# NoSuchThingAsRandom/EpidemicSimulator

Hardware: AMD Instinct MI355X
Metric: citizen-timesteps/sec (higher is better)
Workload: dtype u32 citizen word; u32 uniform vs ceil(q*2^32) (reference: f64 uniform; tolerance 2^-32 per draw); 1 GPU; uk64m: 64000000 citizens, 290000 Output Areas, 10 seeds, steps 1..667 of 5000, interventions on; seed=1592598545

## Files before the change

### epidemicsimulator_amd/csrc/esim_chunk_sets.h

```cpp
#pragma once
#include "esim_kernels_common.h"
#define IV_VALID   0x80000000u
#define IV_PT      (1u << 14)
#define IV_HW      (1u << 15)
#define IV_AS_WORK (1u << 16)
__device__ __forceinline__ uint32_t iv_present(uint32_t iv, uint32_t j, const Decision &q)
{
    if (!(iv & IV_VALID) || j < (iv & 127u) || j > ((iv >> 7) & 127u)) return 0u;
    if (q.bus_dir && (iv & IV_PT)) return 0u;
    const bool at_work = q.at_work && (iv & IV_HW);
    return ((iv & IV_AS_WORK) != 0u) == at_work ? 1u : 0u;
}

__device__ __forceinline__ uint32_t status_in_chunk(const Dev &d, uint32_t w, uint32_t t0, uint32_t j)
{
    const uint32_t f = CW_VAX_REL(w);
    if (f != CW_VAX_NONE && j > f) return ESIM_VACCINATED;
    return status_of(CW_TE(w), t0 + j, d.exposed_time, d.infected_time);
}

__device__ __forceinline__ uint32_t where_in_step(const Dev &d, uint32_t w, uint32_t t0, uint32_t j, const Decision &q)
{
    if (status_in_chunk(d, w, t0, j) != ESIM_INFECTED) return 0u;
    if (q.bus_dir && (w & FL_USES_PT)) return 4u;
    return (q.at_work && (w & FL_HAS_WORK)) ? 2u : 1u;
}

#define FX(x, i) ((uint32_t)__builtin_amdgcn_readlane((int)(x), (int)(i)))
struct M96 { unsigned long long lo; uint32_t hi; };
__device__ __forceinline__ M96 m96_and(M96 a, M96 b) { return M96{ a.lo & b.lo, a.hi & b.hi }; }
__device__ __forceinline__ M96 m96_andn(M96 a, M96 b) { return M96{ a.lo & ~b.lo, a.hi & ~b.hi }; }
__device__ __forceinline__ bool m96_any(M96 a) { return a.lo != 0ull || a.hi != 0u; }
__device__ __forceinline__ M96 m96_range(uint32_t a, uint32_t b)
{
    M96 r = { 0ull, 0u };
    if (a < 64u) { const uint32_t e = min(b, 63u); r.lo = (e == 63u ? ~0ull : ((1ull << (e + 1u)) - 1ull)) & (~0ull << a); }
    if (b >= 64u) { const uint32_t s0 = a > 64u ? a - 64u : 0u, e = min(b - 64u, 31u); r.hi = (e == 31u ? ~0u : ((1u << (e + 1u)) - 1u)) & (~0u << s0); }
    return r;
// ... 61 lines not shown
```

### epidemicsimulator_amd/csrc/esim_device.h

```cpp
#pragma once
#include <stdint.h>

#define CW_TE_SHIFT    19u
#define CW_BUS_EXPOSED (1u << 18)
#define CW_FLAGS       0xFFu
#define CW_VAX_SHIFT   11u
#define CW_VAX_MASK    (0x7Fu << CW_VAX_SHIFT)
#define CW_KEEP        (CW_FLAGS | CW_VAX_MASK)
#define CW_VAX_NONE    0xFFFFFFFFu
#define CW_PLAN_SKIP   (1u << 10)
#define CW_VAX_REL(w)  ((((w) >> CW_VAX_SHIFT) & 0x7Fu) ? 127u - (((w) >> CW_VAX_SHIFT) & 0x7Fu) : CW_VAX_NONE)
#define CW_VAX_FIELD(j) ((127u - (j)) << CW_VAX_SHIFT)
#define CW_TE(w)       ((w) >> CW_TE_SHIFT)
#define CW_MAKE(te, rest) (((te) << CW_TE_SHIFT) | (rest))
#define TE_SUSCEPTIBLE 0x1FFFu
#define TE_VACCINATED  0x1FFEu
#define TE_RECOVERED   0x1FFDu
#define TE_BIAS        512u
#define TE_SLOTS       8192u
#define ESIM_MAX_STEP  7600u

#define FL_USES_PT        0x01u
#define FL_MASK_COMPLIANT 0x02u
#define FL_SAME_AREA      0x04u
// ... 47 lines not shown
    uint32_t prev_cut;
    uint32_t prev_n, prev_n_eff, prev_vax;
    uint32_t vax_cuts;
    uint32_t vax_planned, prev_planned;
    uint32_t xs_need;
    uint32_t xs_need_all;
    uint32_t vax_fail;
    uint32_t err_where;
    uint32_t peer_error;
    uint32_t quiet;
    uint32_t chunk_bus;
    uint32_t replan_from;
    uint32_t repair_ran;
    uint32_t vax_repairs;
};

#define ERR_FIELD(code) ((code) ? 1u << (5u * (((code) < 1u || (code) > 6u ? 6u : (code)) - 1u)) : 0u)
#define ERR_MAX_WORLD 31u
#define XE_WORDS (2u + ERR_MAX_WORLD)
static inline __host__ __device__ uint32_t err_decode(uint32_t word)
{
    for (uint32_t c = 1u; c <= 6u; ++c) if ((word >> (5u * (c - 1u))) & 31u) return c;
    return word ? 6u : 0u;
}

struct UnitRec { uint32_t slot, link, lo, n_mem, code, own, m_first, pad; };

struct BldRec { uint32_t res_lo, res_hi, wrk_lo, wrk_hi, type, ovf_lo, ovf_hi, pad; };
#define SD_REPL 8u

struct ItemRec { uint32_t id, a_lo, a_hi, b_lo, b_hi, aux, link, own; };
#define CHUNK_WAVES_MAX 4096u
#define SLOT_COUNTERS_ONLY 0x40000000u
#ifndef ITEM_RECS
#define ITEM_RECS 7u
#define SLOT_IV_STRIDE 8u
#endif
#define LANE_STATE 24u
#define LANE_HSLOT 25u

struct Decision {
    uint32_t lockdown;
    uint32_t mask;
    uint32_t at_work, bus_dir;
};

struct Dev {
    uint32_t n;
    uint32_t n_global;
    uint32_t id_base;
    uint32_t n_bld, n_room, n_pt;
    uint32_t *cit;
    const uint32_t *home, *work, *room;
    const uint32_t *res_off, *res_idx;
    const uint32_t *wrk_off, *wrk_idx;
    const uint32_t *room_off, *room_idx;
    const uint32_t *room_bld;
    const uint8_t  *bld_type;
    uint32_t *cnt_bld[MARK_SLOTS];
    uint32_t *cnt_room[MARK_SLOTS];
    uint32_t *touched_bld[MARK_SLOTS], *touched_room[MARK_SLOTS], *touched_route[MARK_SLOTS], *touched_route_big[MARK_SLOTS];
    uint32_t *route_flag[MARK_SLOTS];
    uint32_t *exp_step;
    uint32_t *exp_part;
    struct Decision *dec;
    unsigned long long *hkey;
    uint32_t hcap;
    uint32_t *hitems;
    struct ItemRec *item_rec;
    uint32_t *slot_state;
    uint32_t *slot_iv;
    uint32_t *vec;
    uint32_t items_cap;
    struct UnitRec *units;
    uint32_t *route_pairs;
    uint32_t *pair_cnt;
    uint32_t *used_cnt;
    uint32_t *route_pairs_big;
    uint32_t big_pairs_cap;
    const uint32_t *ovf_off;
    uint32_t ovf_room_base;
    uint32_t *ovf;
    uint32_t ovf_n;
    uint32_t n_wrk_idx, n_room_idx;
    const int32_t *sch_of_bld;
    uint32_t n_sch;
    uint32_t *sch_diff;
    const uint4 *where4;
    const struct BldRec *bld8;
    uint32_t *big_list;
    uint32_t big_qcap;
    uint32_t *used_pref;
    uint32_t unit_qcap;
    uint32_t *newexp;
    uint32_t newexp_cap;
    uint32_t *hot;
    uint32_t *cursor;
    uint32_t max_route;
    uint32_t *vax_ev;
    uint32_t *vax_cnt;
    uint32_t *vax_now;
    uint32_t *lost_list;
    uint32_t *vax_delta;
    uint32_t *xf_adj;
    uint32_t *hist;
    uint32_t *log;
    uint32_t *log_off;
    const uint64_t *thr;
    Ctrl *ctrl;
    struct esim_step_result *records;
    uint32_t n_routes;
    const uint32_t *route_off;
    const uint32_t *route_riders;
    const uint32_t *route_of;
    uint32_t *bus_key; uint32_t *bus_idx; uint32_t *bus_cnt; uint8_t *bus_flag;
    uint32_t exposed_time, infected_time, vaccination_rate, bus_capacity, start_hour, end_hour;
    uint32_t seed_lo, seed_hi;
    double thr_lockdown, thr_vacc, thr_mask_pt, thr_mask_all;
    uint32_t max_steps;
    uint32_t n_shards;
    uint32_t n_shared_bld, n_shared_room;
// ... 58 lines not shown
```

### epidemicsimulator_amd/csrc/esim_host_upload.h

```cpp
namespace {

struct UploadHost {
    const esim_population *pop;
    uint32_t N, B, R, n_global;
    bool sharded;
    std::vector<uint8_t> fl;
    std::vector<uint32_t> room_fixed;
    std::vector<uint32_t> route_off, riders, route_of;
    uint32_t n_routes = 0, max_route = 0, n_big_routes = 0;
    bool any_big = false;
    std::vector<uint32_t> res_off, res_idx, wrk_off, wrk_idx, room_off, room_idx;
    bool home_sorted = true;
};

int upload_validate(esim_ctx_impl *c, UploadHost &u)
{
    const esim_population *pop = u.pop; const uint32_t N = u.N, B = u.B, R = u.R;
    if (!pop->home_building || !pop->work_building || !pop->room || !pop->flags || !pop->building_area || !pop->building_type)
        return fail(c, ESIM_EINVAL, "esim_upload_population: a required array is NULL");
    if (R && !pop->room_building) return fail(c, ESIM_EINVAL, "esim_upload_population: room_building is NULL");
    if (pop->n_seeds && !pop->seeds) return fail(c, ESIM_EINVAL, "esim_upload_population: seeds is NULL");
    u.n_global = pop->n_citizens_global ? pop->n_citizens_global : N;
    if ((uint64_t)pop->citizen_id_base + N > u.n_global) return fail(c, ESIM_EINVAL, "esim_upload_population: shard range exceeds n_citizens_global");
    u.sharded = u.n_global != N || pop->n_shared_buildings || pop->n_shared_rooms;
// ... 156 lines not shown
    if ((rc = dev_alloc_fill(c, &d.item_rec, d.items_cap))) return rc;
    if ((rc = dev_alloc_fill(c, &d.vec, (size_t)cap * FREE_MAX))) return rc;
    if ((rc = dev_alloc_fill(c, &d.slot_state, cap))) return rc;
    if ((rc = dev_alloc_fill(c, &d.slot_iv, (size_t)cap * SLOT_IV_STRIDE))) return rc;
    size_t units = 0;
    auto add_lists = [&](const std::vector<uint32_t> &off) {
        for (size_t i = 0; i + 1 < off.size(); ++i) {
            const size_t pairs = (size_t)(off[i + 1] - off[i]) * FREE_MAX;
            if (pairs > UNIT_INLINE) units += (pairs + UNIT_PAIRS - 1) / UNIT_PAIRS;
        }
    };
    add_lists(u.res_off); add_lists(u.wrk_off); add_lists(u.room_off);
    units = std::min<size_t>(units, (size_t)N / 8u + 65536u);
    d.unit_qcap = (uint32_t)std::max<size_t>(1024, units * 2u / SUBQ);
    if ((rc = dev_alloc_fill(c, &d.units, (size_t)d.unit_qcap * SUBQ, 0xFF))) return rc;
    if ((rc = dev_alloc_fill(c, &d.route_pairs, (size_t)d.items_cap * (CHUNK_BUS_STEPS / 4u)))) return rc;
    d.big_pairs_cap = (uint32_t)std::max<size_t>(1, std::min<size_t>((size_t)d.items_cap / 4u, u.n_big_routes) * CHUNK_BUS_STEPS);
    if ((rc = dev_alloc_fill(c, &d.route_pairs_big, d.big_pairs_cap))) return rc;
    std::vector<uint32_t> sch_members((size_t)B + 1, 0);
    for (uint32_t i = 0; i < N; ++i) if (u.fl[i] & FL_WORK_SCHOOL) sch_members[pop->work_building[i] + 1]++;
    for (uint32_t b = 0; b < B; ++b) sch_members[b + 1] += sch_members[b];
    std::vector<uint32_t> ovf_off(u.res_off.size());
    for (size_t i = 0; i < u.res_off.size(); ++i) ovf_off[i] = u.res_off[i] + u.wrk_off[i] + sch_members[i];
    if ((rc = dev_upload(c, &d.ovf_off, ovf_off.data(), ovf_off.size()))) return rc;
    {
        std::vector<int32_t> sch_of(B ? B : 1, -1);
        uint32_t n_sch = 0;
        for (uint32_t b = 0; b < B; ++b) if (pop->building_type[b] == ESIM_SCHOOL) sch_of[b] = (int32_t)n_sch++;
        d.n_sch = n_sch;
        if ((rc = dev_upload(c, &d.sch_of_bld, sch_of.data(), sch_of.size()))) return rc;
    }
    {
        std::vector<uint4> w4(N ? N : 1);
        for (uint32_t i = 0; i < N; ++i) w4[i] = make_uint4(pop->home_building[i], pop->work_building[i], u.room_fixed[i], u.route_of[i]);
        if ((rc = dev_upload(c, &d.where4, w4.data(), w4.size()))) return rc;
        std::vector<BldRec> b8(B ? B : 1);
        for (uint32_t b = 0; b < B; ++b) b8[b] = BldRec{ u.res_off[b], u.res_off[b + 1], u.wrk_off[b], u.wrk_off[b + 1], (uint32_t)pop->building_type[b], ovf_off[b], ovf_off[b + 1], 0u };
        if ((rc = dev_upload(c, &d.bld8, b8.data(), b8.size()))) return rc;
        if ((rc = dev_alloc_fill(c, &d.sch_diff, (size_t)(d.n_sch ? d.n_sch : 1) * SD_REPL * 2u * FREE_MAX))) return rc;
    }
    d.ovf_room_base = ovf_off.back();
    d.ovf_n = d.ovf_room_base + u.room_off.back() + 1u;
    if ((rc = dev_alloc_fill(c, &d.ovf, (size_t)d.ovf_n))) return rc;
    d.n_wrk_idx = (uint32_t)u.wrk_idx.size(); d.n_room_idx = (uint32_t)u.room_idx.size();
    d.big_qcap = d.items_cap / SUBQ;
    if ((rc = dev_alloc_fill(c, &d.big_list, (size_t)d.big_qcap * SUBQ * 3u))) return rc;
    if ((rc = dev_alloc_fill(c, &d.used_pref, CHUNK_WAVES_MAX + 1u))) return rc;
    if ((rc = dev_alloc_fill(c, &d.pair_cnt, 16384u)) || (rc = dev_alloc_fill(c, &d.used_cnt, 16384u))) return rc;
    if ((rc = dev_alloc_fill(c, &d.hot, (size_t)HOT_COUNT * HOT_STRIDE))) return rc;
    d.newexp_cap = N / SUBQ + 1u;
    if ((rc = dev_alloc_fill(c, &d.newexp, (size_t)d.newexp_cap * SUBQ))) return rc;
    if ((rc = dev_alloc_fill(c, &d.cursor, (size_t)EXP_ROWS * FREE_MAX))) return rc;
    return ESIM_OK;
}

int upload_step_tables(esim_ctx_impl *c, const UploadHost &u)
{
    const uint32_t N = u.N, B = u.B, R = u.R;
    Dev &d = c->d; int rc;
    const size_t per_parity = (size_t)B + R + u.n_routes;
    for (int p = 0; p < (int)MARK_SLOTS; ++p) {
        uint32_t *base = c->cnt_base + p * per_parity;
        d.cnt_bld[p] = base; d.cnt_room[p] = base + B; d.route_flag[p] = base + B + R;
        if ((rc = dev_alloc(c, &d.touched_bld[p], B)) || (rc = dev_alloc(c, &d.touched_room[p], R))) return rc;
        if ((rc = dev_alloc(c, &d.touched_route[p], u.n_routes)) || (rc = dev_alloc(c, &d.touched_route_big[p], u.n_routes))) return rc;
    }
    if ((rc = dev_alloc(c, &d.vax_ev, (size_t)FREE_MAX * VACC_MAX_RATE))) return rc;
// ... 268 lines not shown
```

### epidemicsimulator_amd/csrc/esim_kernels_common.h

```cpp
#pragma once
#include <hip/hip_runtime.h>
#include "../../include/esim.h"
#include "esim_device.h"
#include "philox.h"

#define TPB 256
#define FIN_TPB 1024

__device__ __forceinline__ uint32_t status_of(uint32_t te, uint32_t t, uint32_t et, uint32_t it)
{
    if (te == TE_SUSCEPTIBLE) return ESIM_SUSCEPTIBLE;
    if (te == TE_VACCINATED) return ESIM_VACCINATED;
    if (te == TE_RECOVERED) return ESIM_RECOVERED;
    uint32_t d = t + TE_BIAS - te;
    if (d <= et) return ESIM_EXPOSED;
    if (d <= et + 1u + it) return ESIM_INFECTED;
    return ESIM_RECOVERED;
}

__device__ __forceinline__ uint32_t ld(const uint32_t *p)
{
    return __hip_atomic_load(p, __ATOMIC_RELAXED, __HIP_MEMORY_SCOPE_AGENT);
}

// ... 73 lines not shown
#ifdef ESIM_WAVE_PROFILE
#define PROF_ROW 16u
#define PROF_NOW() ((uint32_t)wall_clock64())
#define PROF_PUT(d, i, v) do { if ((threadIdx.x & 63u) == 0) (d).prof_buf[(size_t)(((blockIdx.x * TPB + threadIdx.x) >> 6)) * PROF_ROW + (i)] = (uint32_t)(v); } while (0)
#define BOOKS_PROF(d, i, v) do { if (threadIdx.x == 0) (d).prof_buf[(size_t)16383 * PROF_ROW + (i)] = (uint32_t)(v); } while (0)
#define TINY_PROF(d, i) do { if (threadIdx.x == 0) (d).prof_buf[(size_t)16382 * PROF_ROW + (i)] = (uint32_t)wall_clock64(); } while (0)
#else
#define BOOKS_PROF(d, i, v) do { (void)sizeof(v); } while (0)
#define TINY_PROF(d, i) do { } while (0)
#define PROF_NOW() 0u
#define PROF_PUT(d, i, v) do { (void)sizeof(v); } while (0)
#endif


#ifdef ESIM_COUNT_WORK
enum { WK_ENTRIES = 0,
       WK_KEYS,
       WK_CLAIMS,
       WK_RECORDS,
       WK_DIRECT,
       WK_FOLDED,
       WK_ITEMS,
       WK_MEMBERS,
       WK_MEMBERS_IDX,
       WK_PAIRS,
       WK_PAIRS_ACTIVE,
       WK_BLOCKS,
       WK_DRAWS,
       WK_UNITS,
       WK_ROUTE_PAIRS,
       WK_RIDERS,
       WK_BUS_DRAWS,
       WK_HITS,
       WK_N };
#define WORK_TALLY uint32_t wk_[WK_N]; for (int wk_i = 0; wk_i < WK_N; ++wk_i) wk_[wk_i] = 0u
#define WORK_ADD(i, x) (wk_[i] += (uint32_t)(x))
#define WORK_FLUSH(d) do { for (int wk_i = 0; wk_i < WK_N; ++wk_i) { uint32_t x_ = wk_[wk_i]; for (int o_ = 32; o_ > 0; o_ >>= 1) x_ += __shfl_xor(x_, o_, 64); \
        if ((threadIdx.x & 63u) == 0 && x_) atomicAdd(&(d).work_cnt[wk_i], (unsigned long long)x_); wk_[wk_i] = 0u; } } while (0)
#define WORK_ARG , uint32_t *wk_
#define WORK_PASS , wk_
#else
#define WORK_TALLY do { } while (0)
#define WORK_ADD(i, x) do { } while (0)
#define WORK_FLUSH(d) do { } while (0)
#define WORK_ARG
#define WORK_PASS
#endif
```

### epidemicsimulator_amd/csrc/esim_kernels_draw.h

```cpp
#pragma once
#include "esim_kernels_common.h"
#include "esim_rank.h"
#include "esim_chunk_sets.h"
#include "esim_kernels_marks.h"
__device__ __forceinline__ void expose_min(const Dev &d, Ctrl *ctrl, uint32_t m, uint32_t w, uint32_t s, uint32_t bus)
{
    const uint32_t cand = CW_MAKE(s + TE_BIAS, bus | (w & CW_KEEP));
    const uint32_t prev = atomicMin(&d.cit[m], cand);
    if (bus && cand < prev && CW_VAX_REL(w) != CW_VAX_NONE) {
        const uint32_t at = atomicAdd(&d.hot[HOT_LOST * HOT_STRIDE], 1u);
        if (at < LOST_CAP) d.lost_list[at] = m;
    }
    if (cand < prev && CW_TE(prev) == TE_SUSCEPTIBLE) {
        const uint32_t r = m & (SUBQ - 1u);
        d.newexp[(size_t)r * d.newexp_cap + atomicAdd(&d.hot[(HOT_NEWEXP + r) * HOT_STRIDE], 1u)] = m;
    }
}

struct ChunkShared {
    Decision dec[FREE_MAX];
    uint64_t thr[512];
};
__device__ __forceinline__ void stage_chunk(const Dev &d, ChunkShared &sm, uint32_t n, uint32_t n_threads)
{
// ... 104 lines not shown
        for (uint32_t h = 0; h < SLOT_STEPS; ++h) {
            const int j = j0 + (int)h;
            const uint32_t jc = (uint32_t)(j < 0 ? 0 : j >= (int)FREE_MAX ? (int)FREE_MAX - 1 : j);
            c[h] = ws.cnt[jc]; sc[h] = ws.sch[jc];
        }
        uint32_t nn = 0u, ns = 0u;
#pragma unroll
        for (uint32_t h = 0; h < SLOT_STEPS; ++h) {
            if (!((mk >> h) & 1u)) c[h] = 0u;
            nn |= (c[h] & 255u) << (8u * h);
            ns |= (sc[h] & 255u) << (8u * h);
        }
        const uint32_t i = (uint32_t)__popcll(present & ((1ull << lane) - 1ull));
        ws.desc[2u * i] = make_uint4((uint32_t)(j0 + 3) | (mk << 8) | (m96_nibble(AW, j0) << 12) | (m96_nibble(EV, j0) << 16), nn, ns,
                                     min(c[0], 0xFFFFu) | (min(c[1], 0xFFFFu) << 16));
        ws.desc[2u * i + 1u] = make_uint4(min(c[2], 0xFFFFu) | (min(c[3], 0xFFFFu) << 16), 0u, 0u, 0u);
    }
    return (uint32_t)__popcll(present);
}

__device__ __forceinline__ void school_counts(const Dev &d, uint32_t s_sch, uint32_t lane, uint32_t n, WaveScratch &ws)
{
    uint32_t c0 = 0u, c1 = 0u;
    if (s_sch != 0xFFFFFFFFu) {
        if (lane < n) c0 = d.vec[(size_t)s_sch * FREE_MAX + lane];
        if (64u + lane < n) c1 = d.vec[(size_t)s_sch * FREE_MAX + 64u + lane];
    }
    put_school(ws, lane, c0, c1);
}

struct UnitSrc { uint32_t slot, link, own; };
__device__ __forceinline__ void list_or_units(const Dev &d, Ctrl *ctrl, const ChunkShared &sm, WaveScratch &ws, const uint32_t *idx,
                                              uint32_t lo, uint32_t hi, const UnitSrc &src, uint32_t lane, uint32_t kind, uint32_t S, uint32_t t0 WORK_ARG,
                                              bool have_pre = false, uint32_t pre_m = 0u, uint32_t pre_w = 0u)
{
    const uint32_t pairs = (hi - lo) * S;
    if (pairs == 0) return;
    if (pairs <= UNIT_INLINE) { member_pairs(d, ctrl, sm, ws, idx, lo, 0u, pairs, lane, kind, S, t0 WORK_PASS, have_pre, pre_m, pre_w); return; }
    const uint32_t n_units = (pairs + UNIT_PAIRS - 1u) / UNIT_PAIRS;
    const uint32_t r = ((blockIdx.x * TPB + threadIdx.x) >> 6) & (SUBQ - 1u);
    uint32_t start = 0;
    if (lane == 0) start = atomicAdd(&d.hot[(HOT_UNITS + r) * HOT_STRIDE], n_units);
    start = __shfl(start, 0, 64);
    UnitRec *q = d.units + (size_t)r * d.unit_qcap;
    if (start + n_units > d.unit_qcap) {
        for (uint32_t i = lane; i < n_units && start + i < d.unit_qcap; i += 64u) q[start + i].code = UNIT_NOOP;
        member_pairs(d, ctrl, sm, ws, idx, lo, 0u, pairs, lane, kind, S, t0 WORK_PASS, have_pre, pre_m, pre_w);
        return;
    }
    for (uint32_t i = lane; i < n_units; i += 64u) {
        const uint32_t p_lo = i * UNIT_PAIRS;
        q[start + i] = UnitRec{ src.slot, kind == 2u ? src.link : 0xFFFFFFFFu, lo, hi - lo, (kind << 30) | p_lo, src.own, p_lo / S, 0u };
    }
}

struct ItemFetch { uint32_t slot, id, a_lo, a_hi, b_lo, b_hi, aux, link, c0, c1; };
__device__ __forceinline__ uint32_t fetch_item(const Dev &d, uint32_t v, uint32_t lane)
{
    uint32_t x = 0u;
    if (lane < 8u) x = reinterpret_cast<const uint32_t *>(d.item_rec)[(size_t)v * 8u + lane];
    else if (lane == LANE_HSLOT) x = d.hitems[v];
    return x;
}
__device__ __forceinline__ uint32_t fetch_slot(const Dev &d, uint32_t slot, uint32_t lane)
{
    uint32_t x = 0u;
    if (slot < d.hcap) {
        if (lane >= 8u && lane < 8u + ITEM_RECS) x = d.slot_iv[(size_t)slot * SLOT_IV_STRIDE + (lane - 8u)];
        else if (lane == LANE_STATE) x = d.slot_state[slot];
    }
    return x;
}
__device__ __forceinline__ uint32_t merge_fetch(uint32_t by_id, uint32_t by_slot, uint32_t lane)
{
    return (lane < 8u || lane == LANE_HSLOT) ? by_id : by_slot;
}

__device__ __forceinline__ void item_counts(const Dev &d, uint32_t x, uint32_t slot, uint32_t lane, uint32_t n, const M96 &AW,
                                            const M96 &BUS, uint32_t &c0, uint32_t &c1)
{
    const uint32_t state = FX(x, LANE_STATE);
    c0 = 0u; c1 = 0u;
    if (state > ITEM_RECS) {
        if (lane < n) c0 = d.vec[(size_t)slot * FREE_MAX + lane];
        if (64u + lane < n) c1 = d.vec[(size_t)slot * FREE_MAX + 64u + lane];
    }
    const uint32_t n_rec = state >= SLOT_COUNTERS_ONLY ? 0u : state < ITEM_RECS ? state : ITEM_RECS;
    for (uint32_t k = 0; k < n_rec; ++k) {
        const uint32_t iv = (uint32_t)__builtin_amdgcn_readlane((int)x, (int)(8u + k));
        iv_count(iv, lane, AW, BUS, c0, c1);
    }
}

__device__ __forceinline__ ItemFetch decode_item(const Dev &d, uint32_t x, uint32_t lane, uint32_t n, const M96 &AW, const M96 &BUS)
{
    ItemFetch f;
    f.slot = FX(x, LANE_HSLOT); f.id = FX(x, 0); f.a_lo = FX(x, 1); f.a_hi = FX(x, 2); f.b_lo = FX(x, 3); f.b_hi = FX(x, 4); f.aux = FX(x, 5); f.link = FX(x, 6);
    f.c0 = 0u; f.c1 = 0u;
    if (f.slot < d.hcap) {
        item_counts(d, x, f.slot, lane, n, AW, BUS, f.c0, f.c1);
        iv_count(FX(x, 7), lane, AW, BUS, f.c0, f.c1);
    }
    return f;
}

__device__ __forceinline__ bool item_ok(const Dev &d, const ItemFetch &it)
{
    if (it.slot >= d.hcap) return false;
    if (it.id < d.n_bld) return it.a_lo <= it.a_hi && it.a_hi <= d.n && it.b_lo <= it.b_hi && it.b_hi <= d.n_wrk_idx;
    if (it.id < d.n_bld + d.n_room) return it.a_lo <= it.a_hi && it.a_hi <= d.n_room_idx && (it.link == 0xFFFFFFFFu || it.link < d.hcap);
    return true;
}
#define PAIR_SPREAD 1237u
__device__ __forceinline__ void route_pair_small(const Dev &d, Ctrl *ctrl, const ChunkShared &sm, uint32_t off, uint32_t sz, uint32_t j, uint32_t t0, uint32_t lane WORK_ARG)
{
    const uint64_t seed = ((uint64_t)d.seed_hi << 32) | d.seed_lo;
    const uint32_t s = t0 + j, mask = sm.dec[j].mask;
    uint32_t c = 0, w = 0, key = 0;
    bool inf = false;
    WORK_ADD(WK_ROUTE_PAIRS, lane == 0 ? 1 : 0); WORK_ADD(WK_RIDERS, lane < sz ? 1 : 0);
    bool can = false;
    if (lane < sz) {
        c = d.route_riders[off + lane];
        w = d.cit[c];
        inf = status_in_chunk(d, w, t0, j) == ESIM_INFECTED;
        can = rider_can(w, s, j);
    }
    if (!__any(inf) || !__any(can)) return;
    const uint32_t cap = d.bus_capacity;
    uint32_t rank = 0;
    if (sz > cap) {
        if (lane < sz) key = philox4x32_10(d.id_base + c, s, ESIM_SLOT_BUS_ORDER, 0u, d.seed_lo, d.seed_hi).w0;
        rank = rank_wave64(key, lane, sz);
    }
// ... 100 lines not shown
        ow = ow_base + (uint32_t)__popcll(__ballot(ow_base + lane < n_mw && win <= i)) - 1u;
    };
    seek(d_lo);
    auto id_of = [&](uint32_t i) -> uint32_t {
        for (;;) {
            const uint32_t rel = ow - ow_base;
            if (rel == 63u) { ow_base = ow; win = d.used_pref[min(ow_base + lane, n_mw)]; continue; }
            if (ow + 1u < n_mw && (uint32_t)__builtin_amdgcn_readlane((int)win, (int)(rel + 1u)) <= i) { ++ow; continue; }
            return ow * per_wave + (i - (uint32_t)__builtin_amdgcn_readlane((int)win, (int)rel));
        }
    };
    uint32_t id_cur = 0u, id_nxt = 0u, sl_cur = 0u;
    if (d_lo < d_hi) id_cur = fetch_item(d, id_of(d_lo), lane);
    if (d_lo + 1u < d_hi) id_nxt = fetch_item(d, id_of(d_lo + 1u), lane);
    const uint32_t K = PAIR_K(per_wave, ld(&ctrl->chunk_bus));
    const uint32_t w_base = wave % n_mw, w_rep = wave / n_mw;
    uint32_t code_l = 0u, off_l = 0u, sz_l = 0u; bool have = false;
    auto deal = [&](uint32_t k0) {
        const uint32_t k = (k0 + lane) * G + w_rep;
        have = false;
        if (k < K) {
            const uint32_t src = (w_base + n_mw - (uint32_t)(((unsigned long long)k * PAIR_SPREAD) % n_mw)) % n_mw;
            code_l = d.route_pairs[(size_t)src * K + k];
            have = k < d.pair_cnt[src] && (code_l >> 7) < d.n_routes && (code_l & 127u) < n;
        }
    };
    auto deal_riders = [&]() { if (have) { const uint32_t r = code_l >> 7; off_l = d.route_off[r]; sz_l = d.route_off[r + 1] - off_l; } };
    deal(0u);
    stage_chunk(d, sm, n, TPB);
    __syncthreads();
    const uint32_t route_base = d.n_bld + d.n_room;
    WaveScratch &ws = wsc[threadIdx.x >> 6];
    const auto [AW, BUS, EV] = chunk_masks(sm.dec, lane, n);
    if (d_lo < d_hi) sl_cur = fetch_slot(d, FX(id_cur, LANE_HSLOT), lane);
    deal_riders();
#ifdef ESIM_WAVE_PROFILE
    if (lane == 0) ws.rounds = 0u;
#endif
    uint32_t pst[5] = { 0u, 0u, 0u, 0u, 0u };
    const uint32_t pt1 = PROF_NOW();
    for (uint32_t v = d_lo; v < d_hi; ++v) {
        const uint32_t x = merge_fetch(id_cur, sl_cur, lane);
        id_cur = id_nxt;
        if (v + 2u < d_hi) id_nxt = fetch_item(d, id_of(v + 2u), lane);
        if (v + 1u < d_hi) sl_cur = fetch_slot(d, FX(id_cur, LANE_HSLOT), lane);
        const uint32_t pq0 = PROF_NOW();
        const ItemFetch it = decode_item(d, x, lane, n, AW, BUS);
        if (it.slot == ITEM_UNUSED) continue;
        if (!item_ok(d, it)) { if (lane == 0) RAISE(ctrl, ESIM_ERANGE, ERR_AT_ITEM_CHECK); continue; }
        if (it.id >= route_base) continue;
        const uint32_t pi0 = PROF_NOW();
        pst[0] += pi0 - pq0;
        (void)pi0; ++p_items; WORK_ADD(WK_ITEMS, lane == 0 ? 1 : 0);
        if (it.id < d.n_bld) {
            if (it.aux == ESIM_SCHOOL) continue;
            const uint32_t n_res = it.a_hi - it.a_lo, n_wrk = it.b_hi - it.b_lo;
            uint32_t rm = 0u, wm = 0u, rw = 0u, ww = 0u;
            if (lane < n_res) rm = d.res_idx ? d.res_idx[it.a_lo + lane] : it.a_lo + lane;
            if (lane < n_wrk) wm = d.wrk_idx[it.b_lo + lane];
            if (lane < n_res) rw = d.cit[rm];
            if (lane < n_wrk) ww = d.cit[wm];
            const uint32_t pq1 = PROF_NOW();
            const uint32_t S = item_steps_regs(it.c0, it.c1, lane, ws, t0, AW, EV);
            __builtin_amdgcn_wave_barrier();
            const uint32_t pq2 = PROF_NOW();
            const UnitSrc src = { it.slot, it.link, FX(x, 7) };
            list_or_units(d, ctrl, sm, ws, d.res_idx, it.a_lo, it.a_hi, src, lane, 0u, S, t0 WORK_PASS, true, rm, rw);
            const uint32_t pq3 = PROF_NOW();
            list_or_units(d, ctrl, sm, ws, d.wrk_idx, it.b_lo, it.b_hi, src, lane, 1u, S, t0 WORK_PASS, true, wm, ww);
            const uint32_t pq4 = PROF_NOW();
            pst[1] += pq1 - pi0; pst[2] += pq2 - pq1; pst[3] += pq3 - pq2; pst[4] += pq4 - pq3;
        } else {
            const uint32_t n_mem = it.a_hi - it.a_lo;
            uint32_t mm = 0u, mw = 0u;
            if (lane < n_mem) mm = d.room_idx[it.a_lo + lane];
            school_counts(d, it.link, lane, n, ws);
            if (lane < n_mem) mw = d.cit[mm];
            const uint32_t S = item_steps_regs(it.c0, it.c1, lane, ws, t0, AW, EV);
            __builtin_amdgcn_wave_barrier();
            const UnitSrc src = { it.slot, it.link, FX(x, 7) };
            list_or_units(d, ctrl, sm, ws, d.room_idx, it.a_lo, it.a_hi, src, lane, 2u, S, t0 WORK_PASS, true, mm, mw);
        }
        __builtin_amdgcn_wave_barrier();
        { const uint32_t dt = PROF_NOW() - pi0; p_item_max = dt > p_item_max ? dt : p_item_max; }
    }
    const uint32_t pt2 = PROF_NOW();
    for (uint32_t k0 = 0; k0 * G < K; k0 += 64u) {
        if (k0) { deal(k0); deal_riders(); }
        unsigned long long todo = __ballot(have);
        while (todo) {
            const int src_lane = __ffsll((long long)todo) - 1;
            todo &= todo - 1ull;
            const uint32_t code = __shfl(code_l, src_lane, 64), off = __shfl(off_l, src_lane, 64), sz = __shfl(sz_l, src_lane, 64);
            route_pair_small(d, ctrl, sm, off, sz, code & 127u, t0, lane WORK_PASS);
        }
    }
    WORK_FLUSH(d);
    const uint32_t pt3 = PROF_NOW();
#ifndef ESIM_PROFILE_UNITS
    PROF_PUT(d, 0, pt0); PROF_PUT(d, 1, pt1); PROF_PUT(d, 2, pt2); PROF_PUT(d, 3, pt3);
    PROF_PUT(d, 4, p_items); PROF_PUT(d, 5, p_item_max); PROF_PUT(d, 6, wsc[threadIdx.x >> 6].rounds);
    PROF_PUT(d, 11, pst[0]); PROF_PUT(d, 12, pst[1]); PROF_PUT(d, 13, pst[2]); PROF_PUT(d, 14, pst[3]); PROF_PUT(d, 15, pst[4]);
#endif
    (void)pst;
    (void)pt0; (void)pt1; (void)pt2; (void)pt3; (void)p_items; (void)p_item_max;
}

__global__ __launch_bounds__(TPB) void k_chunk_units(Dev d)
{
    __shared__ ChunkShared sm;
    __shared__ WaveScratch wsc[TPB / 64];
    __shared__ RouteShared rs;
    Ctrl *ctrl = d.ctrl;
    const uint32_t t0 = ctrl->chunk_t0, n = ctrl->chunk_ok;
// ... 67 lines not shown
```

### epidemicsimulator_amd/csrc/esim_kernels_marks.h

```cpp
#pragma once
#include "esim_kernels_common.h"
#include "esim_chunk_sets.h"
__device__ __forceinline__ uint32_t hash64(unsigned long long k)
{
    k ^= k >> 33; k *= 0xff51afd7ed558ccdull; k ^= k >> 33; k *= 0xc4ceb9fe1a85ec53ull; k ^= k >> 33;
    return (uint32_t)k;
}

#define ITEM_UNUSED 0xFFFFFFFFu

__global__ __launch_bounds__(TPB) void k_chunk_marks(Dev d)
{
    Ctrl *ctrl = d.ctrl;
    const uint32_t t0 = ctrl->chunk_t0, n = ctrl->chunk_ok;
    if (!ctrl->chunk_parallel || n == 0u) return;
    clear_marks(d, ctrl, (t0 + MARK_SLOTS - 1u) & (MARK_SLOTS - 1u), blockIdx.x * TPB + threadIdx.x, gridDim.x * TPB);
    const uint32_t lane = threadIdx.x & 63u;
    const uint32_t wave = (blockIdx.x * TPB + threadIdx.x) >> 6, n_waves = (gridDim.x * TPB) >> 6;
    const uint32_t i0 = ctrl->chunk_i0, i1 = ctrl->chunk_i1;
    uint32_t n_remote = 0u;
    if (d.world > 1u) for (uint32_t r = 0; r < d.world; ++r) if (r != d.rank) n_remote += min(d.xs[(size_t)r * (1u + 3u * d.xs_cap)], d.xs_cap);
    const uint32_t per_wave = 4u * ((i1 - i0 + n_remote + n_waves - 1u) / n_waves + (n_remote ? 1u : 0u));
    if (wave == 0 && lane == 0) { ctrl->items_per_wave = per_wave; ctrl->n_items = per_wave * n_waves; }
    if ((unsigned long long)per_wave * n_waves > d.items_cap) { if (lane == 0) ctrl->error = (uint32_t)(-ESIM_ERANGE); return; }
// ... 12 lines not shown
        const uint32_t idx = wave + n_waves * (round * 64u + lane);
        bool act = idx < total;
        const bool remote = act && idx >= E;
        uint32_t c = 0u, w = 0u, r_bld = 0xFFFFFFFFu, r_room = 0xFFFFFFFFu;
        if (act && !remote) { c = d.log[i0 + idx]; w = d.cit[c]; }
        if (remote) {
            uint32_t e = idx - E;
            const uint32_t *seg = nullptr;
            for (uint32_t r = 0; r < d.world; ++r) {
                if (r == d.rank) continue;
                const uint32_t *sg = d.xs + (size_t)r * (1u + 3u * d.xs_cap);
                const uint32_t cnt = min(sg[0], d.xs_cap);
                if (e < cnt) { seg = sg; break; }
                e -= cnt;
            }
            act = false;
            if (seg) {
                w = seg[1u + 3u * e];
                const uint32_t sb = seg[2u + 3u * e], sr = seg[3u + 3u * e];
                const int32_t lb = d.shared_bld[sb];
                if (lb >= 0) {
                    act = true;
                    r_bld = (uint32_t)lb;
                    const int32_t lr = sr != 0xFFFFFFFFu ? d.shared_room[sr] : -1;
                    if (lr >= 0) r_room = (uint32_t)lr;
                }
            }
        }
        const Stretch st = infected_stretch(d, w, t0, n, AW, BUS, act);
        const bool any_home = !remote && m96_any(st.home), any_work = m96_any(st.work), any_bus = !remote && m96_any(st.bus);
        const bool school = w & FL_WORK_SCHOOL;
        if (any_home || any_work || any_bus) { ++p_entries; WORK_ADD(WK_ENTRIES, 1); }
        uint32_t src[4] = { 0u, r_bld, r_room, 0u };
        if (!remote && (any_home || any_work || any_bus)) {
            const uint4 k4 = d.where4[c];
            src[0] = k4.x; src[1] = k4.y; src[2] = k4.z; src[3] = k4.w;
        }
        unsigned long long key[4];
        key[0] = any_home ? (unsigned long long)src[0] : HKEY_EMPTY;
        key[1] = any_work ? (unsigned long long)src[1] : HKEY_EMPTY;
        key[2] = (any_work && school && src[2] != 0xFFFFFFFFu) ? (unsigned long long)d.n_bld + src[2] : HKEY_EMPTY;
        key[3] = any_bus ? (unsigned long long)d.n_bld + d.n_room + src[3] : HKEY_EMPTY;
        const uint32_t pb = PROF_NOW() + (uint32_t)(key[0] & 0ull) + (uint32_t)(key[1] & 0ull) + (uint32_t)(key[2] & 0ull) + (uint32_t)(key[3] & 0ull);
        uint32_t slot[4];
        unsigned long long seen[4];
#pragma unroll
        for (uint32_t k = 0; k < 4u; ++k) {
            slot[k] = hash64(key[k]) & (d.hcap - 1u);
            seen[k] = key[k];
            if (key[k] != HKEY_EMPTY) seen[k] = d.hkey[slot[k]];
        }
#pragma unroll
        for (uint32_t k = 0; k < 4u; ++k)
            if (key[k] != HKEY_EMPTY && seen[k] == HKEY_EMPTY) seen[k] = atomicCAS(&d.hkey[slot[k]], HKEY_EMPTY, key[k]);
        bool claimed[4], pending[4];
#pragma unroll
        for (uint32_t k = 0; k < 4u; ++k) {
            claimed[k] = false; pending[k] = false;
            if (key[k] == HKEY_EMPTY) continue;
            WORK_ADD(WK_KEYS, 1);
            if (seen[k] == HKEY_EMPTY) claimed[k] = true;
            else if (seen[k] == key[k]) pending[k] = true;
            else {
                uint32_t h = slot[k];
                bool found = false;
                for (uint32_t probe = 1; probe < d.hcap && !found; ++probe) {
                    h = (h + 1u) & (d.hcap - 1u);
                    const unsigned long long old = atomicCAS(&d.hkey[h], HKEY_EMPTY, key[k]);
                    if (old == HKEY_EMPTY) { claimed[k] = true; found = true; }
                    else if (old == key[k]) { pending[k] = true; found = true; }
                }
                if (!found) { ctrl->error = (uint32_t)(-ESIM_ERANGE); key[k] = HKEY_EMPTY; h = 0u; }
                slot[k] = h;
            }
        }
        const uint32_t pc = PROF_NOW() + (slot[0] & 0u) + (slot[1] & 0u) + (slot[2] & 0u) + (slot[3] & 0u);
        const uint32_t iv_home = stretch_record(st, w);
        const uint32_t iv_work = iv_home | IV_AS_WORK;
        uint32_t before = 0u, n_claims = 0u;
#pragma unroll
        for (uint32_t k = 0; k < 4u; ++k) { const unsigned long long cm = __ballot(claimed[k]); before += (uint32_t)__popcll(cm & lt); n_claims += (uint32_t)__popcll(cm); }
#pragma unroll
        for (uint32_t k = 0; k < 4u; ++k) {
            if (claimed[k]) {
                WORK_ADD(WK_CLAIMS, 1);
                const uint32_t v = next_id + before++;
                d.hitems[v] = slot[k];
                const uint32_t id = (uint32_t)key[k];
                ItemRec rec = { id, 0u, 0u, 0u, 0u, 0u, k == 2u ? slot[1] : 0xFFFFFFFFu,
                                k == 0u ? iv_home : (k == 1u && !school) || k == 2u ? iv_work : 0u };
                if (k == 0u || k == 1u) {
                    const uint4 b4 = *reinterpret_cast<const uint4 *>(&d.bld8[id]);
                    rec.a_lo = b4.x; rec.a_hi = b4.y; rec.b_lo = b4.z; rec.b_hi = b4.w;
                    rec.aux = d.bld8[id].type;
                } else if (k == 2u) {
                    const uint32_t r = id - d.n_bld;
                    rec.a_lo = d.room_off[r]; rec.a_hi = d.room_off[r + 1u];
                    rec.aux = d.room_bld[r];
                }
                d.item_rec[v] = rec;
            }
        }
        next_id += n_claims;
        const uint32_t pd = PROF_NOW();
        uint32_t mine = 0u;
        if (any_bus) {
            uint32_t i = 0u;
            for (unsigned long long m = BUS.lo; m; m &= m - 1ull, ++i) mine |= (uint32_t)((st.bus.lo >> __builtin_ctzll(m)) & 1ull) << i;
            for (uint32_t m = BUS.hi; m; m &= m - 1u, ++i) mine |= ((st.bus.hi >> __builtin_ctz(m)) & 1u) << i;
        }
        bool add_rec[3];
        uint32_t old[4] = { 0u, 0u, 0u, 0u };
#pragma unroll
        for (uint32_t k = 0; k < 3u; ++k) {
            add_rec[k] = pending[k] && !(k == 1u && school);
            if (add_rec[k]) old[k] = atomicAdd(&d.slot_state[slot[k]], 1u);
        }
        if (claimed[1] && school) d.slot_state[slot[1]] = SLOT_COUNTERS_ONLY;
        if (any_bus && key[3] != HKEY_EMPTY) old[3] = atomicOr(&d.slot_state[slot[3]], mine);
        bool direct[3], first[3];
        uint32_t first_base[3] = { 0u, 0u, 0u }, first_cap[3] = { 0u, 0u, 0u };
        if (school && key[1] != HKEY_EMPTY) {
            const int32_t sch = d.sch_of_bld[(uint32_t)key[1]];
            if (sch < 0 || (uint32_t)sch >= d.n_sch) RAISE(ctrl, ESIM_ERANGE, ERR_AT_SCHOOL);
            else {
                uint32_t *dd = d.sch_diff + ((size_t)sch * SD_REPL + (wave & (SD_REPL - 1u))) * 2u * FREE_MAX;
                WORK_ADD(WK_DIRECT, (w & FL_USES_PT) ? 4 : 2);
                atomicAdd(&dd[st.iv_a], 1u);
                if (st.iv_b + 1u < FREE_MAX) atomicAdd(&dd[st.iv_b + 1u], 0xFFFFFFFFu);
                if (w & FL_USES_PT) {
                    atomicAdd(&dd[FREE_MAX + st.iv_a], 1u);
                    if (st.iv_b + 1u < FREE_MAX) atomicAdd(&dd[FREE_MAX + st.iv_b + 1u], 0xFFFFFFFFu);
                }
                if (claimed[1]) { first_base[1] = (uint32_t)sch; first_cap[1] = 0xFFFFFFFFu; }
            }
        }
#pragma unroll
        for (uint32_t k = 0; k < 3u; ++k) {
            direct[k] = false; first[k] = k == 1u && first_cap[1] == 0xFFFFFFFFu;
            if (!add_rec[k]) continue;
            WORK_ADD(WK_RECORDS, 1);
            const uint32_t iv = k == 0u ? iv_home : iv_work;
            if (old[k] < ITEM_RECS) { d.slot_iv[(size_t)slot[k] * SLOT_IV_STRIDE + old[k]] = iv; continue; }
            const uint32_t q = old[k] - ITEM_RECS, id = (uint32_t)key[k];
            uint32_t base, cap;
            if (k < 2u) { base = d.bld8[id].ovf_lo; cap = d.bld8[id].ovf_hi - base; }
            else { const uint32_t r = id - d.n_bld; const uint32_t o = d.room_off[r]; base = d.ovf_room_base + o; cap = d.room_off[r + 1u] - o; }
            if (q < cap) { d.ovf[base + q] = iv; first[k] = q == 0u; first_base[k] = base; first_cap[k] = cap; }
            else direct[k] = true;
        }
        {
            const unsigned long long f[3] = { __ballot(first[0]), __ballot(first[1]), __ballot(first[2]) };
            const uint32_t n_first = (uint32_t)(__popcll(f[0]) + __popcll(f[1]) + __popcll(f[2]));
            if (n_first) {
                const uint32_t r = wave & (SUBQ - 1u);
                uint32_t at0 = 0u;
                if (lane == 0) at0 = atomicAdd(&d.hot[(HOT_BIG + r) * HOT_STRIDE], n_first);
                at0 = __shfl(at0, 0, 64);
                uint32_t *bl = d.big_list + (size_t)r * d.big_qcap * 3u;
                uint32_t at = at0;
#pragma unroll
                for (uint32_t k = 0; k < 3u; ++k) {
                    const uint32_t pos = at + (uint32_t)__popcll(f[k] & lt);
                    if (first[k] && pos < d.big_qcap) { bl[3u * pos] = slot[k]; bl[3u * pos + 1u] = first_base[k]; bl[3u * pos + 2u] = first_cap[k]; }
                    at += (uint32_t)__popcll(f[k]);
                }
                if (at0 + n_first > d.big_qcap && lane == 0) ctrl->error = (uint32_t)(-ESIM_ERANGE);
            }
        }
#pragma unroll
        for (uint32_t k = 0; k < 3u; ++k) {
            const M96 at = k == 0u ? st.home : st.work;
            for (unsigned long long sp = __ballot(direct[k]); sp; sp &= sp - 1ull) {
                const int src_lane = __builtin_ctzll(sp);
// ... 184 lines not shown
```

### epidemicsimulator_amd/csrc/esim_kernels_tiny.h

```cpp
#pragma once
#include "esim_kernels_common.h"
#include "esim_chunk_sets.h"
#include "esim_kernels_plan.h"
#include "esim_kernels_draw.h"
#include "esim_kernels_books.h"

#define TINY_E 64u
#define TINY_WAVES (FIN_TPB / 64u)
#define TINY_INLINE 256u
#define TINY_TASKS 512u
#define TINY_BUS 8u
#define TINY_BIG 512u
#define TINY_NONE 0xFFFFFFFFu
#define TINY_SYNC() do { __builtin_amdgcn_fence(__ATOMIC_RELEASE, "workgroup"); __syncthreads(); __builtin_amdgcn_fence(__ATOMIC_ACQUIRE, "agent"); } while (0)

struct TinyShared {
    uint32_t e_c[TINY_E], e_w[TINY_E], e_iv[TINY_E];
    __attribute__((aligned(16))) uint32_t e_key[TINY_E][4];
    uint32_t uniq[4u * TINY_E];
    uint32_t n_uniq, n_tasks, n_big;
    uint32_t task[TINY_TASKS][3];
    uint32_t big[TINY_BIG];
};
static_assert(TINY_BIG >= TINY_E * TINY_BUS, "k_chunk_tiny: every entry's route on every bus step the guard admits must fit big[]");
// ... 42 lines not shown
        TINY_SYNC();
    }
    TINY_PROF(d, 2);
    const uint32_t t0 = ld(&ctrl->chunk_t0), n = ld(&ctrl->chunk_ok);
    const uint32_t i0 = ld(&ctrl->chunk_i0), i1 = ld(&ctrl->chunk_i1);
    const uint32_t E = i1 - i0;
    bool run = ld(&ctrl->chunk_parallel) != 0u && n != 0u;
    const unsigned long long key_space = (unsigned long long)d.n_bld + d.n_room + d.n_routes;
    if (run && (i1 < i0 || E > TINY_E || ld(&ctrl->vax_chunk) != 0u || ld(&ctrl->have_elig) != 0u || d.world > 1u || ld(&ctrl->chunk_bus) > TINY_BUS || key_space >= 0xFFFFFFFFull || n > FREE_MAX)) {
        __syncthreads();
        if (tid == 0) ctrl->chunk_parallel = 0u;
        TINY_SYNC();
        run = false;
    }
    if (run) {
        WORK_TALLY;
        clear_marks(d, ctrl, (t0 + MARK_SLOTS - 1u) & (MARK_SLOTS - 1u), tid, FIN_TPB);
        stage_chunk(d, sm, n, FIN_TPB);
        if (tid == 0) { ts.n_uniq = 0u; ts.n_tasks = 0u; ts.n_big = 0u; }
        __syncthreads();
        TINY_PROF(d, 3);
        const auto [AW, BUS, EV] = chunk_masks(sm.dec, lane, n);
        if (tid < TINY_E) {
            uint32_t c = 0u, w = 0u, iv = 0u, key[4] = { TINY_NONE, TINY_NONE, TINY_NONE, TINY_NONE };
            if (tid < E) {
                c = d.log[i0 + tid];
                if (c < d.n) {
                    w = d.cit[c];
                    const Stretch st = infected_stretch(d, w, t0, n, AW, BUS);
                    const bool any_home = m96_any(st.home), any_work = m96_any(st.work), any_bus = m96_any(st.bus);
                    if (any_home || any_work || any_bus) {
                        WORK_ADD(WK_ENTRIES, 1);
                        const uint4 k4 = d.where4[c];
                        if (any_home) key[0] = k4.x;
                        if (any_work) key[1] = k4.y;
                        if (any_work && (w & FL_WORK_SCHOOL) && k4.z != 0xFFFFFFFFu) key[2] = d.n_bld + k4.z;
                        if (any_bus) key[3] = d.n_bld + d.n_room + k4.w;
                        iv = stretch_record(st, w);
                    }
                }
            }
            ts.e_c[tid] = c; ts.e_w[tid] = w; ts.e_iv[tid] = iv;
            ts.e_key[tid][0] = key[0]; ts.e_key[tid][1] = key[1]; ts.e_key[tid][2] = key[2]; ts.e_key[tid][3] = key[3];
        }
        __syncthreads();
        TINY_PROF(d, 4);
        if (tid < 4u * TINY_E) {
            const uint32_t key = (&ts.e_key[0][0])[tid];
            bool first = key != TINY_NONE;
            const uint32_t me = tid >> 2, mk = tid & 3u;
            for (uint32_t e = 0; e <= me && first; ++e) {
                const uint4 k4 = *reinterpret_cast<const uint4 *>(&ts.e_key[e][0]);
                const uint32_t upto = e < me ? 4u : mk;
                if ((upto > 0u && k4.x == key) || (upto > 1u && k4.y == key) || (upto > 2u && k4.z == key) || (upto > 3u && k4.w == key)) first = false;
            }
            if (first) { WORK_ADD(WK_KEYS, 1); ts.uniq[atomicAdd(&ts.n_uniq, 1u)] = key; }
        }
        __syncthreads();
        TINY_PROF(d, 5);
        WaveScratch &ws = wsc[wv];
        const uint32_t n_uniq = ts.n_uniq, route_base = d.n_bld + d.n_room;
        for (uint32_t u = wv; u < n_uniq; u += TINY_WAVES) {
            const uint32_t key = ts.uniq[u];
            if (key >= route_base) {
                const uint32_t r = key - route_base;
                if (r >= d.n_routes) { if (lane == 0) RAISE(ctrl, ESIM_ERANGE, ERR_AT_ROUTE_ITEM); continue; }
                M96 ride = { 0ull, 0u };
                for (uint32_t e = 0; e < E; ++e) if (ts.e_key[e][3] == key) { const uint32_t iv = ts.e_iv[e]; const M96 I = m96_range(iv & 127u, (iv >> 7) & 127u); ride.lo |= I.lo & BUS.lo; ride.hi |= I.hi & BUS.hi; }
                const uint32_t off = d.route_off[r], sz = d.route_off[r + 1u] - off;
// ... 77 lines not shown
```

Before: 56620 billion citizen-timesteps/s.

## Recompute infected counts in-wave for small buildings and rooms instead of storing records

```diff
diff --git a/epidemicsimulator_amd/csrc/esim_chunk_sets.h b/epidemicsimulator_amd/csrc/esim_chunk_sets.h
--- a/epidemicsimulator_amd/csrc/esim_chunk_sets.h
+++ b/epidemicsimulator_amd/csrc/esim_chunk_sets.h
@@ -4,6 +4,7 @@
 #define IV_PT      (1u << 14)
 #define IV_HW      (1u << 15)
 #define IV_AS_WORK (1u << 16)
+#define IV_REMOTE  (1u << 17)
 __device__ __forceinline__ uint32_t iv_present(uint32_t iv, uint32_t j, const Decision &q)
 {
     if (!(iv & IV_VALID) || j < (iv & 127u) || j > ((iv >> 7) & 127u)) return 0u;
diff --git a/epidemicsimulator_amd/csrc/esim_device.h b/epidemicsimulator_amd/csrc/esim_device.h
--- a/epidemicsimulator_amd/csrc/esim_device.h
+++ b/epidemicsimulator_amd/csrc/esim_device.h
@@ -103,6 +103,10 @@
 struct ItemRec { uint32_t id, a_lo, a_hi, b_lo, b_hi, aux, link, own; };
 #define CHUNK_WAVES_MAX 4096u
 #define SLOT_COUNTERS_ONLY 0x40000000u
+#define SMALL_LIST 64u
+#define W4_SMALL 0x80000000u
+static inline __host__ __device__ bool small_building(uint32_t n_res, uint32_t n_wrk, uint32_t type) { return type != (uint32_t)ESIM_SCHOOL && n_res <= SMALL_LIST && n_wrk <= SMALL_LIST; }
+static inline __host__ __device__ bool small_room(uint32_t n_mem) { return n_mem <= SMALL_LIST; }
 #ifndef ITEM_RECS
 #define ITEM_RECS 7u
 #define SLOT_IV_STRIDE 8u
@@ -158,6 +162,7 @@
     uint32_t n_sch;
     uint32_t *sch_diff;
     const uint4 *where4;
+    uint32_t small_on;
     const struct BldRec *bld8;
     uint32_t *big_list;
     uint32_t big_qcap;
diff --git a/epidemicsimulator_amd/csrc/esim_host_upload.h b/epidemicsimulator_amd/csrc/esim_host_upload.h
--- a/epidemicsimulator_amd/csrc/esim_host_upload.h
+++ b/epidemicsimulator_amd/csrc/esim_host_upload.h
@@ -212,7 +212,14 @@
     }
     {
         std::vector<uint4> w4(N ? N : 1);
-        for (uint32_t i = 0; i < N; ++i) w4[i] = make_uint4(pop->home_building[i], pop->work_building[i], u.room_fixed[i], u.route_of[i]);
+        d.small_on = (B < W4_SMALL && u.R < W4_SMALL) ? 1u : 0u;
+        auto bld_bit = [&](uint32_t b) {
+            return d.small_on && small_building(u.res_off[b + 1] - u.res_off[b], u.wrk_off[b + 1] - u.wrk_off[b], pop->building_type[b]) ? W4_SMALL : 0u;
+        };
+        auto room_bit = [&](uint32_t r) { return d.small_on && r < u.R && small_room(u.room_off[r + 1] - u.room_off[r]) ? W4_SMALL : 0u; };
+        for (uint32_t i = 0; i < N; ++i)
+            w4[i] = make_uint4(pop->home_building[i] | bld_bit(pop->home_building[i]), pop->work_building[i] | bld_bit(pop->work_building[i]),
+                               u.room_fixed[i] | room_bit(u.room_fixed[i]), u.route_of[i]);
         if ((rc = dev_upload(c, &d.where4, w4.data(), w4.size()))) return rc;
         std::vector<BldRec> b8(B ? B : 1);
         for (uint32_t b = 0; b < B; ++b) b8[b] = BldRec{ u.res_off[b], u.res_off[b + 1], u.wrk_off[b], u.wrk_off[b + 1], (uint32_t)pop->building_type[b], ovf_off[b], ovf_off[b + 1], 0u };
diff --git a/epidemicsimulator_amd/csrc/esim_kernels_common.h b/epidemicsimulator_amd/csrc/esim_kernels_common.h
--- a/epidemicsimulator_amd/csrc/esim_kernels_common.h
+++ b/epidemicsimulator_amd/csrc/esim_kernels_common.h
@@ -129,6 +129,7 @@
        WK_RIDERS,
        WK_BUS_DRAWS,
        WK_HITS,
+       WK_RECORDS_SMALL,
        WK_N };
 #define WORK_TALLY uint32_t wk_[WK_N]; for (int wk_i = 0; wk_i < WK_N; ++wk_i) wk_[wk_i] = 0u
 #define WORK_ADD(i, x) (wk_[i] += (uint32_t)(x))
diff --git a/epidemicsimulator_amd/csrc/esim_kernels_draw.h b/epidemicsimulator_amd/csrc/esim_kernels_draw.h
--- a/epidemicsimulator_amd/csrc/esim_kernels_draw.h
+++ b/epidemicsimulator_amd/csrc/esim_kernels_draw.h
@@ -160,11 +160,11 @@
 struct UnitSrc { uint32_t slot, link, own; };
 __device__ __forceinline__ void list_or_units(const Dev &d, Ctrl *ctrl, const ChunkShared &sm, WaveScratch &ws, const uint32_t *idx,
                                               uint32_t lo, uint32_t hi, const UnitSrc &src, uint32_t lane, uint32_t kind, uint32_t S, uint32_t t0 WORK_ARG,
-                                              bool have_pre = false, uint32_t pre_m = 0u, uint32_t pre_w = 0u)
+                                              bool have_pre = false, uint32_t pre_m = 0u, uint32_t pre_w = 0u, bool always_here = false)
 {
     const uint32_t pairs = (hi - lo) * S;
     if (pairs == 0) return;
-    if (pairs <= UNIT_INLINE) { member_pairs(d, ctrl, sm, ws, idx, lo, 0u, pairs, lane, kind, S, t0 WORK_PASS, have_pre, pre_m, pre_w); return; }
+    if (pairs <= UNIT_INLINE || always_here) { member_pairs(d, ctrl, sm, ws, idx, lo, 0u, pairs, lane, kind, S, t0 WORK_PASS, have_pre, pre_m, pre_w); return; }
     const uint32_t n_units = (pairs + UNIT_PAIRS - 1u) / UNIT_PAIRS;
     const uint32_t r = ((blockIdx.x * TPB + threadIdx.x) >> 6) & (SUBQ - 1u);
     uint32_t start = 0;
@@ -182,7 +182,7 @@
     }
 }
 
-struct ItemFetch { uint32_t slot, id, a_lo, a_hi, b_lo, b_hi, aux, link, c0, c1; };
+struct ItemFetch { uint32_t slot, id, a_lo, a_hi, b_lo, b_hi, aux, link, c0, c1; bool small; };
 __device__ __forceinline__ uint32_t fetch_item(const Dev &d, uint32_t v, uint32_t lane)
 {
     uint32_t x = 0u;
@@ -198,6 +198,26 @@
         else if (lane == LANE_STATE) x = d.slot_state[slot];
     }
     return x;
+}
+__device__ __forceinline__ bool fetched_small(const Dev &d, uint32_t by_id)
+{
+    const uint32_t id = FX(by_id, 0), n_a = FX(by_id, 2) - FX(by_id, 1);
+    if (!d.small_on || FX(by_id, LANE_HSLOT) >= d.hcap) return false;
+    if (id < d.n_bld) return small_building(n_a, FX(by_id, 4) - FX(by_id, 3), FX(by_id, 5));
+    return id < d.n_bld + d.n_room && small_room(n_a);
+}
+__device__ __forceinline__ uint32_t fetch_slot_of(const Dev &d, uint32_t by_id, uint32_t lane)
+{
+    if (d.world == 1u && fetched_small(d, by_id)) return 0u;
+    return fetch_slot(d, FX(by_id, LANE_HSLOT), lane);
+}
+__device__ __forceinline__ void member_counts(const Dev &d, uint32_t w, bool has, bool as_work, uint32_t t0, uint32_t n, uint32_t lane,
+                                              const M96 &AW, const M96 &BUS, uint32_t &c0, uint32_t &c1)
+{
+    const Stretch st = infected_stretch(d, w, t0, n, AW, BUS, has);
+    const uint32_t iv = stretch_record(st, w) | (as_work ? IV_AS_WORK : 0u);
+    for (unsigned long long todo = __ballot(m96_any(as_work ? st.work : st.home)); todo; todo &= todo - 1ull)
+        iv_count(FX(iv, __builtin_ctzll(todo)), lane, AW, BUS, c0, c1);
 }
 __device__ __forceinline__ uint32_t merge_fetch(uint32_t by_id, uint32_t by_slot, uint32_t lane)
 {
@@ -225,9 +245,10 @@
     ItemFetch f;
     f.slot = FX(x, LANE_HSLOT); f.id = FX(x, 0); f.a_lo = FX(x, 1); f.a_hi = FX(x, 2); f.b_lo = FX(x, 3); f.b_hi = FX(x, 4); f.aux = FX(x, 5); f.link = FX(x, 6);
     f.c0 = 0u; f.c1 = 0u;
+    f.small = fetched_small(d, x);
     if (f.slot < d.hcap) {
         item_counts(d, x, f.slot, lane, n, AW, BUS, f.c0, f.c1);
-        iv_count(FX(x, 7), lane, AW, BUS, f.c0, f.c1);
+        if (!f.small || (FX(x, 7) & IV_REMOTE)) iv_count(FX(x, 7), lane, AW, BUS, f.c0, f.c1);
     }
     return f;
 }
@@ -394,7 +415,7 @@
     const uint32_t route_base = d.n_bld + d.n_room;
     WaveScratch &ws = wsc[threadIdx.x >> 6];
     const auto [AW, BUS, EV] = chunk_masks(sm.dec, lane, n);
-    if (d_lo < d_hi) sl_cur = fetch_slot(d, FX(id_cur, LANE_HSLOT), lane);
+    if (d_lo < d_hi) sl_cur = fetch_slot_of(d, id_cur, lane);
     deal_riders();
 #ifdef ESIM_WAVE_PROFILE
     if (lane == 0) ws.rounds = 0u;
@@ -405,7 +426,7 @@
         const uint32_t x = merge_fetch(id_cur, sl_cur, lane);
         id_cur = id_nxt;
         if (v + 2u < d_hi) id_nxt = fetch_item(d, id_of(v + 2u), lane);
-        if (v + 1u < d_hi) sl_cur = fetch_slot(d, FX(id_cur, LANE_HSLOT), lane);
+        if (v + 1u < d_hi) sl_cur = fetch_slot_of(d, id_cur, lane);
         const uint32_t pq0 = PROF_NOW();
         const ItemFetch it = decode_item(d, x, lane, n, AW, BUS);
         if (it.slot == ITEM_UNUSED) continue;
@@ -423,13 +444,18 @@
             if (lane < n_res) rw = d.cit[rm];
             if (lane < n_wrk) ww = d.cit[wm];
             const uint32_t pq1 = PROF_NOW();
-            const uint32_t S = item_steps_regs(it.c0, it.c1, lane, ws, t0, AW, EV);
+            uint32_t c0 = it.c0, c1 = it.c1;
+            if (it.small) {
+                member_counts(d, rw, lane < n_res, false, t0, n, lane, AW, BUS, c0, c1);
+                member_counts(d, ww, lane < n_wrk, true, t0, n, lane, AW, BUS, c0, c1);
+            }
+            const uint32_t S = item_steps_regs(c0, c1, lane, ws, t0, AW, EV);
             __builtin_amdgcn_wave_barrier();
             const uint32_t pq2 = PROF_NOW();
             const UnitSrc src = { it.slot, it.link, FX(x, 7) };
-            list_or_units(d, ctrl, sm, ws, d.res_idx, it.a_lo, it.a_hi, src, lane, 0u, S, t0 WORK_PASS, true, rm, rw);
+            list_or_units(d, ctrl, sm, ws, d.res_idx, it.a_lo, it.a_hi, src, lane, 0u, S, t0 WORK_PASS, true, rm, rw, it.small);
             const uint32_t pq3 = PROF_NOW();
-            list_or_units(d, ctrl, sm, ws, d.wrk_idx, it.b_lo, it.b_hi, src, lane, 1u, S, t0 WORK_PASS, true, wm, ww);
+            list_or_units(d, ctrl, sm, ws, d.wrk_idx, it.b_lo, it.b_hi, src, lane, 1u, S, t0 WORK_PASS, true, wm, ww, it.small);
             const uint32_t pq4 = PROF_NOW();
             pst[1] += pq1 - pi0; pst[2] += pq2 - pq1; pst[3] += pq3 - pq2; pst[4] += pq4 - pq3;
         } else {
@@ -438,10 +464,12 @@
             if (lane < n_mem) mm = d.room_idx[it.a_lo + lane];
             school_counts(d, it.link, lane, n, ws);
             if (lane < n_mem) mw = d.cit[mm];
-            const uint32_t S = item_steps_regs(it.c0, it.c1, lane, ws, t0, AW, EV);
+            uint32_t c0 = it.c0, c1 = it.c1;
+            if (it.small) member_counts(d, mw, lane < n_mem, true, t0, n, lane, AW, BUS, c0, c1);
+            const uint32_t S = item_steps_regs(c0, c1, lane, ws, t0, AW, EV);
             __builtin_amdgcn_wave_barrier();
             const UnitSrc src = { it.slot, it.link, FX(x, 7) };
-            list_or_units(d, ctrl, sm, ws, d.room_idx, it.a_lo, it.a_hi, src, lane, 2u, S, t0 WORK_PASS, true, mm, mw);
+            list_or_units(d, ctrl, sm, ws, d.room_idx, it.a_lo, it.a_hi, src, lane, 2u, S, t0 WORK_PASS, true, mm, mw, it.small);
         }
         __builtin_amdgcn_wave_barrier();
         { const uint32_t dt = PROF_NOW() - pi0; p_item_max = dt > p_item_max ? dt : p_item_max; }
diff --git a/epidemicsimulator_amd/csrc/esim_kernels_marks.h b/epidemicsimulator_amd/csrc/esim_kernels_marks.h
--- a/epidemicsimulator_amd/csrc/esim_kernels_marks.h
+++ b/epidemicsimulator_amd/csrc/esim_kernels_marks.h
@@ -68,9 +68,12 @@
         const bool school = w & FL_WORK_SCHOOL;
         if (any_home || any_work || any_bus) { ++p_entries; WORK_ADD(WK_ENTRIES, 1); }
         uint32_t src[4] = { 0u, r_bld, r_room, 0u };
+        bool small[3] = { false, false, false };
         if (!remote && (any_home || any_work || any_bus)) {
             const uint4 k4 = d.where4[c];
-            src[0] = k4.x; src[1] = k4.y; src[2] = k4.z; src[3] = k4.w;
+            const uint32_t ids = d.small_on ? ~W4_SMALL : 0xFFFFFFFFu;
+            src[0] = k4.x & ids; src[1] = k4.y & ids; src[2] = k4.z & ids; src[3] = k4.w;
+            small[0] = (k4.x & ~ids) != 0u; small[1] = (k4.y & ~ids) != 0u; small[2] = (k4.z & ~ids) != 0u;
         }
         unsigned long long key[4];
         key[0] = any_home ? (unsigned long long)src[0] : HKEY_EMPTY;
@@ -111,7 +114,7 @@
             }
         }
         const uint32_t pc = PROF_NOW() + (slot[0] & 0u) + (slot[1] & 0u) + (slot[2] & 0u) + (slot[3] & 0u);
-        const uint32_t iv_home = stretch_record(st, w);
+        const uint32_t iv_home = stretch_record(st, w) | (remote ? IV_REMOTE : 0u);
         const uint32_t iv_work = iv_home | IV_AS_WORK;
         uint32_t before = 0u, n_claims = 0u;
 #pragma unroll
@@ -149,7 +152,7 @@
         uint32_t old[4] = { 0u, 0u, 0u, 0u };
 #pragma unroll
         for (uint32_t k = 0; k < 3u; ++k) {
-            add_rec[k] = pending[k] && !(k == 1u && school);
+            add_rec[k] = pending[k] && !(k == 1u && school) && !small[k];
             if (add_rec[k]) old[k] = atomicAdd(&d.slot_state[slot[k]], 1u);
         }
         if (claimed[1] && school) d.slot_state[slot[1]] = SLOT_COUNTERS_ONLY;
@@ -176,6 +179,14 @@
             direct[k] = false; first[k] = k == 1u && first_cap[1] == 0xFFFFFFFFu;
             if (!add_rec[k]) continue;
             WORK_ADD(WK_RECORDS, 1);
+#ifdef ESIM_COUNT_WORK
+            {
+                const uint32_t id = (uint32_t)key[k];
+                const bool sm = k < 2u ? small_building(d.bld8[id].res_hi - d.bld8[id].res_lo, d.bld8[id].wrk_hi - d.bld8[id].wrk_lo, d.bld8[id].type)
+                                       : small_room(d.room_off[id - d.n_bld + 1u] - d.room_off[id - d.n_bld]);
+                WORK_ADD(WK_RECORDS_SMALL, (d.small_on && sm) ? 1 : 0);
+            }
+#endif
             const uint32_t iv = k == 0u ? iv_home : iv_work;
             if (old[k] < ITEM_RECS) { d.slot_iv[(size_t)slot[k] * SLOT_IV_STRIDE + old[k]] = iv; continue; }
             const uint32_t q = old[k] - ITEM_RECS, id = (uint32_t)key[k];
diff --git a/epidemicsimulator_amd/csrc/esim_kernels_tiny.h b/epidemicsimulator_amd/csrc/esim_kernels_tiny.h
--- a/epidemicsimulator_amd/csrc/esim_kernels_tiny.h
+++ b/epidemicsimulator_amd/csrc/esim_kernels_tiny.h
@@ -98,9 +98,10 @@
                     if (any_home || any_work || any_bus) {
                         WORK_ADD(WK_ENTRIES, 1);
                         const uint4 k4 = d.where4[c];
-                        if (any_home) key[0] = k4.x;
-                        if (any_work) key[1] = k4.y;
-                        if (any_work && (w & FL_WORK_SCHOOL) && k4.z != 0xFFFFFFFFu) key[2] = d.n_bld + k4.z;
+                        const uint32_t ids = d.small_on ? ~W4_SMALL : 0xFFFFFFFFu;
+                        if (any_home) key[0] = k4.x & ids;
+                        if (any_work) key[1] = k4.y & ids;
+                        if (any_work && (w & FL_WORK_SCHOOL) && k4.z != 0xFFFFFFFFu) key[2] = d.n_bld + (k4.z & ids);
                         if (any_bus) key[3] = d.n_bld + d.n_room + k4.w;
                         iv = stretch_record(st, w);
                     }
```

After: 57610 billion citizen-timesteps/s (median of 5 runs). 1.7% higher.
